# brownvc/matryodshka

Measured on AMD Instinct MI355X. Metric: novel-view frames/sec, 640x320 ODS->32-sphere MSI infer+render, higher is better.
Workload: dtype f32

## Files before the change

include/msi_hip.h:

```cpp
#ifndef MSI_HIP_H
#define MSI_HIP_H

#include <stddef.h>
#include <stdint.h>

#ifdef __cplusplus
extern "C" {
#endif

#define MSI_OK 0
#define MSI_E_BADARG (-1)
#define MSI_E_LAUNCH (-2)
#define MSI_E_UNSUPPORTED (-3)
#define MSI_E_WORKSPACE (-4)
#define MSI_E_RANGE (-5)

typedef void *msi_stream_t;

const char *msi_version(void);
#define MSI_ABI_VERSION 9
int32_t msi_abi_version(void);
const char *msi_last_error_string(void);
uint32_t msi_crc32c_host(const void *data_host, size_t n, uint32_t crc);

// ... 136 lines not shown
#define MSI_NET_OPT_HEAD_FUSE_LN 3
#define MSI_NET_OPT_NUM_CUS 4
#define MSI_NET_OPT_F32_TILE 5
#define MSI_NET_OPT_F32_TILE_MASK 6
#define MSI_NET_OPT_APPLY_AHEAD 7
#define MSI_NET_OPT_HALO 8
#define MSI_NET_OPT_HALO_SKIP 9
#define MSI_NET_OPT_UNIFORM_SPLIT 10
#define MSI_NET_OPT_BF16_STAGE_RAW 11
#define MSI_NET_OPT_SPLIT_OVERHEAD 12
#define MSI_NET_OPT_BF16_WAVES 13
#define MSI_NET_OPT_F32_SPLIT3 14
#define MSI_NET_OPT_F32_SPLIT_F16 15
#define MSI_NET_OPT_X3_TILE8 16
#define MSI_NET_OPT_X3_ROWPAR 17
#define MSI_NET_OPT_COUNT 18
int msi_net_plan_create(const msi_net_desc *desc, msi_net_plan **out_plan);
void msi_net_plan_destroy(msi_net_plan *plan);
int msi_net_plan_set_option(msi_net_plan *plan, int32_t option, int32_t value);
size_t msi_net_plan_workspace_bytes(const msi_net_plan *plan);
int32_t msi_net_plan_layer_is_normalized(const msi_net_plan *plan, int32_t layer);
int32_t msi_net_plan_layer_kernel(const msi_net_plan *plan, int32_t layer, char *name, size_t name_bytes, int32_t *nblocks,
                                  int32_t *nsplit_tiles);
#define MSI_NET_STATUS_APPLY_AHEAD_TIMEOUT 1
#define MSI_NET_STATUS_LN_OVERFLOW 2
#define MSI_NET_STATUS_LN_UNDERFLOW 4
#define MSI_NET_STATUS_F16_SPLIT_RANGE 8
int32_t msi_net_plan_status(const msi_net_plan *plan, const void *workspace, msi_stream_t stream, int32_t *status_bits);
int32_t msi_net_plan_calibrate(const msi_net_plan *plan, float *packed, const void *net_input, void *workspace, size_t workspace_bytes,
                               msi_stream_t stream, int32_t *layers_changed);
int msi_net_plan_forward(const msi_net_plan *plan, const float *packed, const void *net_input, float *pred,
// ... 18 lines not shown
```

matryodshka_amd/_native.py:

```python
import ctypes
import os
from ctypes import POINTER, Structure, c_char, c_char_p, c_float, c_int32, c_size_t, c_uint64, c_void_p

_HERE = os.path.dirname(os.path.abspath(__file__))
LIB_PATH = os.path.join(_HERE, "libmsi_hip.so")

MSI_OK = 0
MSI_NET_NUM_LAYERS = 18
RENDER_STATUS_ORIGIN_OUTSIDE = 1
MSI_CAMERA_EQUIRECT, MSI_CAMERA_PINHOLE = 0, 1
MSI_ABI_VERSION = 9


class MsiError(RuntimeError):
    pass


class NetDesc(Structure):
    _fields_ = [("batch", c_int32), ("height", c_int32), ("width", c_int32),
                ("in_channels", c_int32), ("num_outputs", c_int32), ("ngf", c_int32),
                ("coord_net", c_int32), ("dtype", c_int32)]


MSI_DTYPE_F32, MSI_DTYPE_BF16 = 0, 1
NET_OPT_FIXUP_KERNEL, NET_OPT_TAILSPLIT, NET_OPT_BIGTILE, NET_OPT_HEAD_FUSE_LN, NET_OPT_NUM_CUS = 0, 1, 2, 3, 4
NET_OPT_F32_TILE, NET_OPT_F32_TILE_MASK, NET_OPT_APPLY_AHEAD, NET_OPT_HALO, NET_OPT_HALO_SKIP = 5, 6, 7, 8, 9
NET_OPT_UNIFORM_SPLIT, NET_OPT_BF16_STAGE_RAW, NET_OPT_SPLIT_OVERHEAD, NET_OPT_BF16_WAVES, NET_OPT_F32_SPLIT3 = 10, 11, 12, 13, 14
NET_OPT_F32_SPLIT_F16 = 15
NET_OPT_X3_TILE8 = 16
NET_OPT_X3_ROWPAR = 17
NET_STATUS_F16_SPLIT_RANGE = 8


class LayerInfo(Structure):
    _fields_ = [("name", c_char * 16), ("kind", c_int32), ("cin", c_int32), ("cout", c_int32),
                ("has_coord", c_int32), ("stride", c_int32), ("rate", c_int32),
                ("in_h", c_int32), ("in_w", c_int32), ("out_h", c_int32), ("out_w", c_int32),
                ("param_offset", c_uint64), ("param_floats", c_uint64),
                ("raw_offset", c_uint64), ("affine_offset", c_uint64), ("ln_scale_offset", c_uint64)]


_P = c_void_p
_I = c_int32

SIGNATURES = {
# ... 113 lines not shown
```

matryodshka_amd/csrc/cnn.hip:

```cpp
#include "cnn_device.h"

namespace {

struct Layer {
  char name[16];
  int kind;
  int cin, cout, has_coord, stride, rate;
  int in_h, in_w, out_h, out_w;
  int src0, src1;
  int c0, c1;
  int ntaps, cpt0, cpt1, ksteps, nclass, npad;
  int wrapt;
  int mh, mw;
  double ln_count;
  size_t param_off, param_floats;
  size_t packed_off;
  size_t packed_w_floats;
  size_t gamma_off, beta_off, coord_off;
  size_t lnscl_off;
  size_t x3_off;
  size_t x2_off;
  size_t raw_off, aff_off;
  size_t act_off;
  size_t sums_off;
// ... 298 lines not shown
             (L.rate == 1 || L.rate == 2);
    Q.halo_s2 = halo_ok && (pl->opt[MSI_NET_OPT_HALO] & 4) && !bf16 && !pl->opt[MSI_NET_OPT_APPLY_AHEAD] && Q.tile == TILE_64x64 &&
                L.kind == MODE_CONV && L.stride == 2 && L.rate == 1 && L.src1 < 0 && L.in_h % 2 == 0 && L.in_w % 2 == 0 &&
                L.out_h % 4 == 0 && L.out_w % 16 == 0 && L.c0 % 32 == 0 && p.pad_t == p.pad_l && (p.pad_t == 0 || p.pad_t == 1) &&
                ((long)(L.out_h / 4) * (L.out_w / 16) * (L.cout / 64) * desc->batch >= 3L * pl->num_cus ||
                 (L.x3_off != 0 && ((pl->opt[MSI_NET_OPT_F32_SPLIT3] >> li) & 1) && !(pl->opt[MSI_NET_OPT_HALO_SKIP] >> 20 & 1)));
    if (Q.halo_s2) Q.halo = 1;
    Q.halo_x3 = Q.halo && !bf16 && L.x3_off != 0 && ((pl->opt[MSI_NET_OPT_F32_SPLIT3] >> li) & 1);
    Q.halo_x2 = Q.halo_x3 && ((pl->opt[MSI_NET_OPT_F32_SPLIT_F16] >> li) & 1);
    Q.x3_th8 = Q.halo_x3 && !Q.halo_x2 && !Q.halo_s2 && L.rate == 1 && L.in_h % 8 == 0 && ((pl->opt[MSI_NET_OPT_X3_TILE8] >> li) & 1) &&
               ((long)(L.in_h / 8) * (L.in_w / 16) * ((L.cout + 63) / 64) * desc->batch >= 3L * pl->num_cus || ((pl->opt[MSI_NET_OPT_X3_TILE8] >> 30) & 1));
    if (Q.halo_x3 && !Q.halo_x2 && Q.halo_s2 && L.out_h % 8 == 0 && ((pl->opt[MSI_NET_OPT_X3_TILE8] >> li) & 1) &&
        ((long)(L.out_h / 8) * (L.out_w / 16) * ((L.cout + 63) / 64) * desc->batch >= 3L * pl->num_cus || ((pl->opt[MSI_NET_OPT_X3_TILE8] >> 30) & 1)))
      Q.x3_th8 = 1;
    if (Q.x3_th8) BM = 128;
    p.row_par = (Q.halo_x3 && !Q.halo_s2 && L.kind == MODE_CONV && L.rate == 2 && L.in_h % 8 == 0 && ((pl->opt[MSI_NET_OPT_X3_ROWPAR] >> li) & 1)) ? 1 : 0;
    int max_split = MAX_SPLIT;
    if (halo_ok && (pl->opt[MSI_NET_OPT_HALO] & 1) && bf16 && !pl->opt[MSI_NET_OPT_APPLY_AHEAD] && L.kind == MODE_CONV && L.stride == 1 && L.src1 < 0 && L.in_w % 16 == 0 &&
        L.c0 % 64 == 0 && bigmode != 0) {
      if (L.cout % 128 == 0 && L.in_h % 8 == 0 && (L.rate == 1 || L.rate == 2)) { Q.halo = 1; Q.hbm = 128; Q.hbn = 128; }
      else if (L.cout == 64 && L.in_h % 16 == 0 && L.rate == 1) { Q.halo = 1; Q.hbm = 256; Q.hbn = 64; }
      if (Q.halo) { BM = Q.hbm; BN = Q.hbn; max_split = 1; }
    }
    if (halo_ok && (pl->opt[MSI_NET_OPT_HALO] & 4) && bf16 && !pl->opt[MSI_NET_OPT_APPLY_AHEAD] && L.kind == MODE_CONV && L.stride == 2 && L.rate == 1 &&
        L.src1 < 0 && L.in_h % 2 == 0 && L.in_w % 2 == 0 && L.out_h % 8 == 0 && L.out_w % 16 == 0 && L.c0 % 64 == 0 && L.cout % 128 == 0 &&
        p.pad_t == p.pad_l && (p.pad_t == 0 || p.pad_t == 1) && bigmode != 0) {
      Q.halo = 1; Q.halo_s2 = 1; Q.hbm = 128; Q.hbn = 128; BM = 128; BN = 128; max_split = 1;
    }
    const bool x3_on = !bf16 && L.x3_off != 0 && ((pl->opt[MSI_NET_OPT_F32_SPLIT3] >> li) & 1);
    Q.halo_t = halo_ok && ((pl->opt[MSI_NET_OPT_HALO] & 2) || (x3_on && pl->opt[MSI_NET_OPT_HALO] != 0)) && !bf16
// ... 339 lines not shown
  pl->opt[MSI_NET_OPT_FIXUP_KERNEL] = 0;
  pl->opt[MSI_NET_OPT_TAILSPLIT] = 1;
  pl->opt[MSI_NET_OPT_BIGTILE] = 1;
  pl->opt[MSI_NET_OPT_HEAD_FUSE_LN] = 1;
  pl->opt[MSI_NET_OPT_NUM_CUS] = pl->num_cus;
  pl->opt[MSI_NET_OPT_APPLY_AHEAD] = 0;
  pl->opt[MSI_NET_OPT_HALO] = 5;
  pl->opt[MSI_NET_OPT_F32_TILE] = 0;
  pl->opt[MSI_NET_OPT_F32_TILE_MASK] = 0;
  pl->opt[MSI_NET_OPT_UNIFORM_SPLIT] = 0;
  pl->opt[MSI_NET_OPT_SPLIT_OVERHEAD] = 0;
  pl->opt[MSI_NET_OPT_BF16_WAVES] = 8;
  pl->opt[MSI_NET_OPT_F32_SPLIT_F16] = 0;
  pl->opt[MSI_NET_OPT_X3_TILE8] = 0x3ffff;
  pl->opt[MSI_NET_OPT_X3_ROWPAR] = 0x3ffff;
  pl->opt[MSI_NET_OPT_F32_SPLIT3] = 0x3ffff;
  pl->opt[MSI_NET_OPT_BF16_STAGE_RAW] = 1;
  int rc = plan_layers(pl);
  if (rc) { delete pl; return rc; }
  *out = pl;
  return MSI_OK;
}

void msi_net_plan_destroy(msi_net_plan *plan) { delete plan; }

int msi_net_plan_set_option(msi_net_plan *plan, int32_t option, int32_t value) {
  MSI_REQUIRE(plan, "net_plan_set_option: null plan");
  MSI_REQUIRE(option >= 0 && option < MSI_NET_OPT_COUNT, "net_plan_set_option: unknown option %d", option);
  if (option == MSI_NET_OPT_NUM_CUS) {
    MSI_REQUIRE(value >= 8 && value <= 4096, "net_plan_set_option: num_cus %d out of range", value);
    plan->num_cus = value;
  }
  if (option == MSI_NET_OPT_BIGTILE) MSI_REQUIRE(value >= 0 && value <= 2, "net_plan_set_option: bigtile %d", value);
  if (option == MSI_NET_OPT_HALO) MSI_REQUIRE(value >= 0 && value <= 7, "net_plan_set_option: halo %d (bit 0 conv, bit 1 conv-transpose, bit 2 stride-2 conv)", value);
  if (option == MSI_NET_OPT_TAILSPLIT) MSI_REQUIRE(value >= 0 && value <= 2, "net_plan_set_option: tailsplit %d", value);
  if (option == MSI_NET_OPT_F32_TILE) MSI_REQUIRE(value >= 0 && value <= 2, "net_plan_set_option: f32 tile %d", value);
  if (option == MSI_NET_OPT_BF16_WAVES) MSI_REQUIRE(value == 4 || value == 8, "net_plan_set_option: bf16 waves %d (4 or 8)", value);
#ifndef MSI_EXPERIMENTS
  if ((option == MSI_NET_OPT_F32_TILE || option == MSI_NET_OPT_F32_TILE_MASK || option == MSI_NET_OPT_APPLY_AHEAD) && value != 0)
    return msi::fail(MSI_E_UNSUPPORTED, "net_plan_set_option: option %d is an experiment this library was not built with "
                     "(MSI_CNN_DEFINES=-DMSI_EXPERIMENTS python -m matryodshka_amd.build --force)", option);
#endif
  const int old = plan->opt[option];
  plan->opt[option] = value;
  int rc = plan_layers(plan);
  if (rc) {
    plan->opt[option] = old;
    if (option == MSI_NET_OPT_NUM_CUS) plan->num_cus = old;
    plan_layers(plan);
  }
  return rc;
}
// ... 17 lines not shown
  const int bf16 = plan->desc.dtype == MSI_DTYPE_BF16;
  const char *mode = L.kind == MODE_CONV ? "0" : (L.kind == MODE_CONVT ? "1" : "2");
  if (Q.halo_tb) {
    snprintf(name, name_bytes, "convt_halo_bf16_kernel<128, %d, %d>", Q.hbn, Q.p.halo_apply ? 1 : 0);
  } else if (Q.halo && bf16) {
    if (Q.halo_s2) snprintf(name, name_bytes, "conv_halo_bf16_s2_kernel<%d, 4>", Q.halo_apply ? 1 : 0);
    else if (Q.hbm == 128) snprintf(name, name_bytes, "conv_halo_bf16_kernel<128, 128, %d, %d, %d>", L.rate, Q.halo_apply ? 1 : 0,
                                    plan->opt[MSI_NET_OPT_BF16_WAVES] == 8 ? 8 : 4);
    else snprintf(name, name_bytes, "conv_halo_bf16_kernel<256, 64, 1, %d, 4>", Q.halo_apply ? 1 : 0);
  } else if (Q.halo_t) {
    if (Q.halo_x3 && Q.x3_th8) snprintf(name, name_bytes, "convt_halo8_x3_kernel");
    else if (Q.halo_x3) snprintf(name, name_bytes, "convt_halo_x3_kernel<%d>", Q.halo_x2 ? 2 : 3);
    else snprintf(name, name_bytes, "convt_halo_kernel");
  } else if (Q.halo) {
    if (Q.halo_s2 && Q.halo_x3 && Q.x3_th8) snprintf(name, name_bytes, "conv_halo8_s2_x3_kernel<%d>", Q.halo_apply ? 1 : 0);
    else if (Q.halo_s2 && Q.halo_x3) snprintf(name, name_bytes, "conv_halo_s2_x3_kernel<%d, %d>", Q.halo_apply ? 1 : 0, Q.halo_x2 ? 2 : 3);
    else if (Q.halo_s2) snprintf(name, name_bytes, "conv_halo_s2_kernel<%d>", Q.halo_apply ? 1 : 0);
    else if (Q.x3_th8) snprintf(name, name_bytes, "conv_halo8_x3_kernel<%d, 3>", Q.halo_apply ? 1 : 0);
    else if (Q.halo_x3) snprintf(name, name_bytes, "conv_halo_x3_kernel<%d, %d, %d>", Q.p.row_par ? 3 : L.rate, Q.halo_apply ? 1 : 0, Q.halo_x2 ? 2 : 3);
    else snprintf(name, name_bytes, "conv_halo_kernel<%d, %d>", L.rate, Q.halo_apply ? 1 : 0);
  } else {
    const int bm = Q.tile == TILE_128x128 || Q.tile == TILE_128x64 ? 128 : 64;
    const int bn = Q.tile == TILE_128x128 || Q.tile == TILE_64x128 ? 128 : 64;
    snprintf(name, name_bytes, "conv_igemm_kernel<%d, %d, %s, %d>", bm, bn, mode, bf16);
  }
  if (nblocks) *nblocks = Q.nblocks + Q.p.n_apply;
  if (nsplit_tiles) *nsplit_tiles = Q.nfix;
  return MSI_OK;
}

#ifdef MSI_DEBUG_SUMS
// ... 316 lines not shown
```

matryodshka_amd/csrc/cnn_device.h:

```cpp
#pragma once
#include <cmath>
#include <cstdint>
#include <cstdio>
#include <cstdlib>
#include <cstring>
#include <new>
#include <type_traits>
#include <vector>

#include "msi_common.h"

namespace msi_cnn {


typedef float f32x16 __attribute__((ext_vector_type(16)));
typedef float v4f __attribute__((ext_vector_type(4)));
typedef __attribute__((address_space(3))) void lds_void;

constexpr int BK = 32;
constexpr int ROW_BYTES = BK * 4;
#ifndef MSI_NSTAGE
#define MSI_NSTAGE 2
#endif
constexpr int NSTAGE = MSI_NSTAGE;
constexpr int NPAD_ALIGN = 128;
constexpr int COORD_CLASSES = 5;
[[maybe_unused]] constexpr unsigned OOB = 0x80000000u;
constexpr int DEFAULT_CUS = 256;
constexpr int MAX_SPLIT = 8;
constexpr int CONV_SLOTS_PER_CU = 5;
constexpr double LN_EPS = 1e-12;
constexpr int LN_SHARDS = 64, LN_WORDS = 2;
constexpr int LN_S1_BITS = 24, LN_S2_BITS = 16;
constexpr int LN_SCL_DOUBLES = 4;
constexpr double LN_UNDERFLOW_UNITS_SQ = 1e12;
enum { STATUS_APPLY_AHEAD_TIMEOUT = 1, STATUS_LN_OVERFLOW = 2, STATUS_LN_UNDERFLOW = 4, STATUS_F16_SPLIT_RANGE = 8 };
constexpr int AP_FLAG_STRIDE = 16;
constexpr int HEAD_MAX_C = 256;

enum { MODE_CONV = 0, MODE_CONVT = 1, MODE_HEAD = 2 };

struct ConvParams {
  const char *x0, *x1;
  const char *wpk;
// ... 45 lines not shown

enum { TILE_64x64 = 0, TILE_128x128 = 1, TILE_128x64 = 2, TILE_64x128 = 3 };

struct LayerLaunch {
  ConvParams p;
  int tile;
  int nblocks, nfix;
  int inlaunch;
  int fuse_ln;
  int skip_apply;
  int halo;
  int halo_s2;
  int halo_x3;
  int halo_x2;
  int x3_th8;
  int hbm, hbn;
  int halo_t;
  int halo_tb;
  int halo_apply;
  unsigned ln_blocks;
};


constexpr int HA_TP = 32;
#ifndef MSI_HA_LG
#define MSI_HA_LG 32
#endif
constexpr int HA_LG = MSI_HA_LG;

struct HeadAsmParams {
// ... 681 lines not shown
```

matryodshka_amd/csrc/cnn_x3.hip:

```cpp
#include "cnn_device.h"

namespace {

#ifndef MSI_X3_EARLY_DMA
#define MSI_X3_EARLY_DMA 0
#endif
#ifndef MSI_X3_NSTG
#define MSI_X3_NSTG 0
#endif
#ifndef MSI_X3_ABLATE
#define MSI_X3_ABLATE 0
#endif
#ifndef MSI_X2_NSTG
#define MSI_X2_NSTG 3
#endif
constexpr int x3_rate_y(int RATE) { return RATE == 3 ? 1 : RATE; }
constexpr int x3_rate_x(int RATE) { return RATE == 3 ? 2 : RATE; }
constexpr int x3_nstg(int RATE, int NPL) { return NPL == 2 ? MSI_X2_NSTG : (MSI_X3_NSTG ? MSI_X3_NSTG : (RATE == 2 ? 3 : 2)); }
template <int RATE, int NS = x3_nstg(RATE, 3), int NPL = 3, int TH = 4>
struct HaloGeomX3 {
  static constexpr int PW = 16 + 2 * x3_rate_x(RATE), PH = TH + 2 * x3_rate_y(RATE), NPX = PW * PH;
  static constexpr int PIX_BYTES = NPL * 64 + 16;
  static constexpr int ROW_PITCH = ((PW * PIX_BYTES + 127) / 256) * 256 + 128;
  static constexpr int A_BYTES = PH * ROW_PITCH;
// ... 408 lines not shown
    v4f r = y - v4f{__builtin_bit_cast(float, h0 << 16), __builtin_bit_cast(float, h0 & 0xffff0000u),
                    __builtin_bit_cast(float, h1 << 16), __builtin_bit_cast(float, h1 & 0xffff0000u)};
    asm("v_cvt_pk_bf16_f32 %0, %1, %2" : "=v"(m0) : "v"(r.x), "v"(r.y));
    asm("v_cvt_pk_bf16_f32 %0, %1, %2" : "=v"(m1) : "v"(r.z), "v"(r.w));
    r = r - v4f{__builtin_bit_cast(float, m0 << 16), __builtin_bit_cast(float, m0 & 0xffff0000u),
                __builtin_bit_cast(float, m1 << 16), __builtin_bit_cast(float, m1 & 0xffff0000u)};
    asm("v_cvt_pk_bf16_f32 %0, %1, %2" : "=v"(l0) : "v"(r.x), "v"(r.y));
    asm("v_cvt_pk_bf16_f32 %0, %1, %2" : "=v"(l1) : "v"(r.z), "v"(r.w));
    if (off != 0xffffffffu) {
      *reinterpret_cast<u2x_t *>(smem + off) = u2x_t{h0, h1};
      *reinterpret_cast<u2x_t *>(smem + off + 64) = u2x_t{m0, m1};
      *reinterpret_cast<u2x_t *>(smem + off + 128) = u2x_t{l0, l1};
    }
  }
}
template <int NP>
__device__ __forceinline__ void split_mfma(f32x16 &acc, f32x16 &lo, const v4f &ah, const v4f &am, const v4f &al, const v4f &bh, const v4f &bm, const v4f &bl) {
  typedef __bf16 bf16x8 __attribute__((ext_vector_type(8)));
  typedef _Float16 f16x8 __attribute__((ext_vector_type(8)));
  if (NP == 2) {
    lo = __builtin_amdgcn_mfma_f32_32x32x16_f16(__builtin_bit_cast(f16x8, bm), __builtin_bit_cast(f16x8, ah), lo, 0, 0, 0);
    acc = __builtin_amdgcn_mfma_f32_32x32x16_f16(__builtin_bit_cast(f16x8, bh), __builtin_bit_cast(f16x8, ah), acc, 0, 0, 0);
    lo = __builtin_amdgcn_mfma_f32_32x32x16_f16(__builtin_bit_cast(f16x8, bh), __builtin_bit_cast(f16x8, am), lo, 0, 0, 0);
  } else {
    acc = __builtin_amdgcn_mfma_f32_32x32x16_bf16(__builtin_bit_cast(bf16x8, bm), __builtin_bit_cast(bf16x8, am), acc, 0, 0, 0);
    acc = __builtin_amdgcn_mfma_f32_32x32x16_bf16(__builtin_bit_cast(bf16x8, bh), __builtin_bit_cast(bf16x8, al), acc, 0, 0, 0);
    acc = __builtin_amdgcn_mfma_f32_32x32x16_bf16(__builtin_bit_cast(bf16x8, bl), __builtin_bit_cast(bf16x8, ah), acc, 0, 0, 0);
    acc = __builtin_amdgcn_mfma_f32_32x32x16_bf16(__builtin_bit_cast(bf16x8, bh), __builtin_bit_cast(bf16x8, am), acc, 0, 0, 0);
    acc = __builtin_amdgcn_mfma_f32_32x32x16_bf16(__builtin_bit_cast(bf16x8, bm), __builtin_bit_cast(bf16x8, ah), acc, 0, 0, 0);
    acc = __builtin_amdgcn_mfma_f32_32x32x16_bf16(__builtin_bit_cast(bf16x8, bh), __builtin_bit_cast(bf16x8, ah), acc, 0, 0, 0);
  }
}
template <int NP>
__device__ __forceinline__ void split_finish(f32x16 &acc, const f32x16 &lo, unsigned amax, int lane, int *status) {
  if (NP == 2) {
#pragma unroll
    for (int r = 0; r < 16; ++r) acc[r] = __builtin_fmaf(lo[r], 1.f / 2048.f, acc[r]);
    if (__builtin_amdgcn_ballot_w64(amax > F16_MAX_BITS) != 0 && lane == 0) atomicOr(status, STATUS_F16_SPLIT_RANGE);
  }
}

#ifndef MSI_S2X3_NSTG
#define MSI_S2X3_NSTG 2
#endif
template <int NP, int TH = 4>
struct HaloGeomS2X3 {
  static constexpr int PW = 17, PH = TH + 1, NPX = PW * PH;
  static constexpr int PIX_BYTES = NP * 64 + 16;
  static constexpr int ROW_PITCH = ((PW * PIX_BYTES + 127) / 256) * 256 + 128;
  static constexpr int A_BYTES = PH * ROW_PITCH;
  static constexpr int B_ROW = 64, B_PLANE = 64 * B_ROW, B_STAGE = NP * B_PLANE;
  static constexpr int NSTG = NP == 3 ? MSI_S2X3_NSTG : 3;
  static constexpr int LDS_BYTES = A_BYTES + NSTG * B_STAGE;
  static constexpr int NLOAD = (NPX * 8 + 255) / 256;
};

#ifndef MSI_S2X_WAVES
#define MSI_S2X_WAVES 3
#ifndef MSI_S2X3_ABLATE
#define MSI_S2X3_ABLATE 0
#endif
#endif
template <int APPLY, int NP, int TH>
__device__ __forceinline__ void conv_halo_s2_x3_body(const ConvParams &p, char *smem) {
  typedef HaloGeomS2X3<NP, TH> G;
  constexpr int PW = G::PW, NPX = G::NPX, NLOAD = G::NLOAD;
  constexpr int MT = TH / 4, NT = 1, BM = 16 * TH;
  static_assert(TH == 4 || (TH == 8 && NP == 3 && G::NSTG == 2), "the 8-row tile: six-product form, two-stage ring");
  const int tid = threadIdx.x, lane = tid & 63;
  const int wave = __builtin_amdgcn_readfirstlane(tid >> 6);
  const int wm = wave >> 1, wn = wave & 1;
  const int CH = p.cpt0;
  int t, c0 = 0, c1 = CH, ks = 0, slot = 0;
  {
    const int bid = blockIdx.x;
    if (bid < p.nb_main && p.split0 == 1) {
      const int q = p.n_main >> 3, r = p.n_main & 7, xcd = bid & 7, local = bid >> 3;
      t = (xcd < r ? xcd * (q + 1) : r * (q + 1) + (xcd - r) * q) + local;
    } else {
      int sp, r, tbase;
      unsigned mg;
      if (bid < p.nb_main) { sp = p.split0; mg = p.mg_sp0; r = bid; tbase = 0; }
      else { sp = p.split; mg = p.mg_sp; r = bid - p.nb_main; tbase = p.n_main; }
// ... 63 lines not shown
      }
      __builtin_amdgcn_sched_barrier(0);
    }
  }

  float inv_f = 1.f, mu_hi = 0.f, mu_lo = 0.f;
  bool has_pad = false;
  if (APPLY) {
    bool bad = false;
#pragma unroll
    for (int k = 0; k < NLOAD; ++k)
#pragma unroll
      for (int u = 0; u < 4; ++u) bad |= (lds_a[k] != 0xffffffffu) && !pok[u][k];
    has_pad = __builtin_amdgcn_ballot_w64(bad) != 0;
  }
  v4f s4 = {1.f, 1.f, 1.f, 1.f}, t4 = {0.f, 0.f, 0.f, 0.f};
  auto patch_load = [&](const int c, auto U_c) __attribute__((always_inline)) {
    constexpr int U = decltype(U_c)::value;
    if (MSI_S2X3_ABLATE & 64) return;
#pragma unroll
    for (int k_ = 0; k_ < NLOAD; ++k_)
      araw[k_] = __builtin_bit_cast(v4f, (u32x4_t)__builtin_amdgcn_raw_buffer_load_b128(rsrc_a, voff[U][k_], c * ROW_BYTES, 0));
    if (APPLY && U == 0) {
      g4 = *reinterpret_cast<const v4f *>(p.ln_gamma + c * 32 + cslot * 4);
      be4 = *reinterpret_cast<const v4f *>(p.ln_beta + c * 32 + cslot * 4);
    }
  };
  auto patch_store = [&](auto U_c) __attribute__((always_inline)) {
    constexpr int U = decltype(U_c)::value;
    if (APPLY && U == 0) {
      s4 = inv_f * g4;
      const v4f nh = {-mu_hi, -mu_hi, -mu_hi, -mu_hi}, nl = {-mu_lo, -mu_lo, -mu_lo, -mu_lo};
      t4 = __builtin_elementwise_fma(nl, s4, __builtin_elementwise_fma(nh, s4, be4));
    }
#pragma unroll
    for (int k_ = 0; k_ < NLOAD; ++k_) {
      v4f y = araw[k_];
      if (APPLY) {
        y = __builtin_elementwise_max(__builtin_elementwise_fma(y, s4, t4), v4f{0.f, 0.f, 0.f, 0.f});
        if (has_pad && !pok[U][k_]) y = v4f{0.f, 0.f, 0.f, 0.f};
      }
// ... 12 lines not shown
  typedef __bf16 bf16x8 __attribute__((ext_vector_type(8), unused));
  f32x16 acc[MT][1], acc_lo;
#pragma unroll
  for (int r = 0; r < 16; ++r) {
    acc_lo[r] = 0.f;
#pragma unroll
    for (int i = 0; i < MT; ++i) acc[i][0][r] = 0.f;
  }

  int c = c0, cpar = 0;
  auto s2step = [&](auto J_c) __attribute__((always_inline)) {
    constexpr int J = decltype(J_c)::value;
    constexpr int TAP_ = s2_tap(J), U_ = s2_unit(J);
    constexpr int DY_ = (TAP_ / 3) >> 1, DX_ = (TAP_ % 3) >> 1;
    constexpr bool FIRST_ = J == 0 || J == 4 || J == 6 || J == 8, LAST_ = J == 3 || J == 5 || J == 7 || J == 8;
    constexpr int AOFF_ = DY_ * G::ROW_PITCH + DX_ * G::PIX_BYTES;
    const bool more_ = U_ < 3 || c + 1 < c1;
    const unsigned bst_ = (unsigned)(G::NSTG == 3 ? J % 3 : ((J ^ cpar) & 1)) * G::B_STAGE;
    if (G::NSTG == 2) {
      const int stn_ = ((J ^ cpar) & 1) ^ 1;
      if (J + 1 < 9) b_issue(c, s2_tap((J + 1) % 9), stn_);
      else if (c + 1 < c1) b_issue(c + 1, s2_tap(0), stn_);
    }
    v4f ah_[2], am_[2], al_[2], bh_[2], bm_[2], bl_[2];
    if constexpr (MT == 2) {
      constexpr int A1_ = AOFF_ + 2 * G::ROW_PITCH;
      v4f xh_[2][2], xm_[2][2], xl_[2][2];
      bh_[0] = lds_read128<0>(b_s[0] + bst_); bm_[0] = lds_read128<G::B_PLANE>(b_s[0] + bst_); bl_[0] = lds_read128<2 * G::B_PLANE>(b_s[0] + bst_);
      xh_[0][0] = lds_read128<AOFF_>(a_base); xm_[0][0] = lds_read128<AOFF_ + 64>(a_base); xl_[0][0] = lds_read128<AOFF_ + 128>(a_base);
      xh_[0][1] = lds_read128<A1_>(a_base); xm_[0][1] = lds_read128<A1_ + 64>(a_base); xl_[0][1] = lds_read128<A1_ + 128>(a_base);
      bh_[1] = lds_read128<0>(b_s[1] + bst_); bm_[1] = lds_read128<G::B_PLANE>(b_s[1] + bst_); bl_[1] = lds_read128<2 * G::B_PLANE>(b_s[1] + bst_);
      wait_lgkm6<6>(bh_[0], bm_[0], bl_[0], xh_[0][0], xm_[0][0], xl_[0][0]);
// ... 15 lines not shown
      split_mfma<3>(acc[1][0], acc_lo, xh_[1][1], xm_[1][1], xl_[1][1], bh_[1], bm_[1], bl_[1]);
      __builtin_amdgcn_sched_barrier(0);
    } else {
    if (!(MSI_S2X3_ABLATE & 8))
#pragma unroll
    for (int s_ = 0; s_ < 2; ++s_) {
      ah_[s_] = s_ == 0 ? lds_read128<AOFF_>(a_base) : lds_read128<AOFF_ + 32>(a_base);
      bh_[s_] = lds_read128<0>(b_s[s_] + bst_);
      am_[s_] = s_ == 0 ? lds_read128<AOFF_ + 64>(a_base) : lds_read128<AOFF_ + 96>(a_base);
      bm_[s_] = lds_read128<G::B_PLANE>(b_s[s_] + bst_);
      if (NP == 3) {
        al_[s_] = s_ == 0 ? lds_read128<AOFF_ + 128>(a_base) : lds_read128<AOFF_ + 160>(a_base);
        bl_[s_] = lds_read128<2 * G::B_PLANE>(b_s[s_] + bst_);
      } else { al_[s_] = ah_[s_]; bl_[s_] = bh_[s_]; }
    }
#pragma unroll
    for (int s_ = 0; s_ < 2; ++s_) {
      if (NP == 3) {
        if (s_ == 0) wait_lgkm6<6>(ah_[0], bh_[0], am_[0], bm_[0], al_[0], bl_[0]);
        else wait_lgkm6<0>(ah_[1], bh_[1], am_[1], bm_[1], al_[1], bl_[1]);
      } else {
        if (s_ == 0) wait_lgkm4<4>(ah_[0], bh_[0], am_[0], bm_[0]);
        else wait_lgkm4<0>(ah_[1], bh_[1], am_[1], bm_[1]);
      }
      if (!(MSI_S2X3_ABLATE & 16)) split_mfma<NP>(acc[0][0], acc_lo, ah_[s_], am_[s_], al_[s_], bh_[s_], bm_[s_], bl_[s_]);
      __builtin_amdgcn_sched_barrier(0);
      if (s_ == 0) {
        if (FIRST_ && more_) {
          if (U_ < 3) patch_load(c, IC<(U_ + 1) & 3>{});
          else patch_load(c + 1, IC<0>{});
        }
        if (G::NSTG == 3) {
        if (J + 2 < 9) b_issue(c, s2_tap((J + 2) % 9), (J + 2) % 3);
        else if (c + 1 < c1) b_issue(c + 1, s2_tap((J + 2) % 9), (J + 2) % 3);
        }
      }
    }
    }
    {
      const bool issued_ = (J + 2 < 9) || (c + 1 < c1);
      if (G::NSTG == 2) {
        if (FIRST_ && !LAST_ && more_) wait_vmcnt<NLOAD>();
        else wait_vmcnt<0>();
      } else if (FIRST_ && !LAST_ && more_) wait_vmcnt<NP + NLOAD>();
      else if (issued_) wait_vmcnt<NP>();
      else wait_vmcnt<0>();
    }
    if (!(MSI_S2X3_ABLATE & 4)) __builtin_amdgcn_s_barrier();
    if (LAST_ && more_ && !(MSI_S2X3_ABLATE & 32)) {
      patch_store(IC<(U_ + 1) & 3>{});
      asm volatile("s_waitcnt lgkmcnt(0)" ::: "memory");
      __builtin_amdgcn_s_barrier();
    }
  };

  if (APPLY) {
    double *s_stat = reinterpret_cast<double *>(smem);
    ln_mean_inv(p.ln_sums + (size_t)b * LN_SHARDS * LN_WORDS, p.ln_inv_n, p.ln_scl_src, p.status, s_stat, tid);
    const double mu = s_stat[0];
    inv_f = (float)s_stat[1];
    mu_hi = (float)mu;
    mu_lo = (float)(mu - (double)mu_hi);
    __syncthreads();
  }
  wait_vmcnt<0>();
  patch_store(IC<0>{});
  asm volatile("s_waitcnt lgkmcnt(0)" ::: "memory");
  __builtin_amdgcn_s_barrier();
  for (; c < c1; ++c) {
    cpar = (c - c0) & 1;
    s2step(IC<0>{}); s2step(IC<1>{}); s2step(IC<2>{}); s2step(IC<3>{}); s2step(IC<4>{});
    s2step(IC<5>{}); s2step(IC<6>{}); s2step(IC<7>{}); s2step(IC<8>{});
  }
  split_finish<NP>(acc[0][0], acc_lo, amax_, lane, p.status);

  if (!full) {
    constexpr int SLAB = BM * 64 * 4;
    const __amdgpu_buffer_rsrc_t rsrc_p = __builtin_amdgcn_make_buffer_rsrc((void *)(p.partial + (size_t)slot * (BM * 64)), 0, SLAB, 0x00020000);
    if (p.tile_cnt == nullptr) {
      dump_acc<MT, NT, 0>(acc, rsrc_p, tid);
      return;
// ... 9 lines not shown
    __syncthreads();
    if (*s_old != nsp - 1) return;
    handoff_acquire();
    const __amdgpu_buffer_rsrc_t rsrc_t = __builtin_amdgcn_make_buffer_rsrc((void *)(p.partial + (size_t)(slot - ks) * (BM * 64)), 0, nsp * SLAB, 0x00020000);
    sum_slabs<MT, NT, MSI_HANDOFF_AUX>(acc, rsrc_t, nsp, SLAB, tid);
    __syncthreads();
  }
  emit_tile<BM, 64, MODE_CONV>(p, acc, tile_m, tile_n, 0, b, tid, smem);
}

template <int APPLY, int NP>
__global__ void __launch_bounds__(256) __attribute__((amdgpu_waves_per_eu(NP == 2 ? MSI_S2X_WAVES : (MSI_S2X3_NSTG == 2 ? 3 : 2))))
conv_halo_s2_x3_kernel(const ConvParams p) {
#if defined(__HIP_DEVICE_COMPILE__)
  extern __shared__ __attribute__((aligned(16))) char smem[];
  conv_halo_s2_x3_body<APPLY, NP, 4>(p, smem);
#endif
}

template <int APPLY>
__global__ void __launch_bounds__(256) __attribute__((amdgpu_waves_per_eu(2)))
conv_halo8_s2_x3_kernel(const ConvParams p) {
#if defined(__HIP_DEVICE_COMPILE__)
  extern __shared__ __attribute__((aligned(16))) char smem[];
  conv_halo_s2_x3_body<APPLY, 3, 8>(p, smem);
#endif
}

template <int NS, int NPL, int TH = 4>
struct HaloGeomCT3 : HaloGeomX3<1, NS, NPL, TH> {
  typedef HaloGeomX3<1, NS, NPL, TH> B_;
// ... 336 lines not shown
  convt_halo_x3_body<3, 8>(p, smem);
#endif
}

}

namespace msi_cnn {
int launch_x3(const LayerLaunch &Q, const ConvParams &p, int rate, hipStream_t stream) {
  const dim3 grid(Q.nblocks), block(256);
  if (Q.halo_t) {
    constexpr int lds_ct3 = HaloGeomCT3<MSI_CT3_NSTG, 3>::LDS_BYTES, lds_ct2 = HaloGeomCT3<3, 2>::LDS_BYTES;
    constexpr int lds_ct8 = HaloGeomCT3<MSI_CT3_NSTG, 3, 8>::LDS_BYTES;
    static_assert(lds_ct8 <= 65536, "convt_halo8_x3_kernel: LDS without the launch attribute");
    if (Q.x3_th8) hipLaunchKernelGGL(convt_halo8_x3_kernel, grid, block, lds_ct8, stream, p);
    else if (Q.halo_x2) hipLaunchKernelGGL(convt_halo_x3_kernel<2>, grid, block, lds_ct2, stream, p);
    else hipLaunchKernelGGL(convt_halo_x3_kernel<3>, grid, block, lds_ct3, stream, p);
    int rc = msi::check_launch("convt_halo_x3");
    if (!rc && Q.nfix > 0 && p.tile_cnt == nullptr) rc = launch_fixup(Q.x3_th8 ? 128 : 64, 64, MODE_CONVT, Q.nfix, 2, p, stream);
    return rc;
  }
  if (Q.halo_s2 && Q.x3_th8) {
    typedef HaloGeomS2X3<3, 8> G8s_;
    static_assert(G8s_::LDS_BYTES <= 65536, "conv_halo8_s2_x3_kernel: LDS without the launch attribute");
    if (Q.halo_apply) hipLaunchKernelGGL((conv_halo8_s2_x3_kernel<1>), grid, block, G8s_::LDS_BYTES, stream, p);
    else hipLaunchKernelGGL((conv_halo8_s2_x3_kernel<0>), grid, block, G8s_::LDS_BYTES, stream, p);
  } else if (Q.halo_s2) {
    if (Q.halo_x2) {
      if (Q.halo_apply) hipLaunchKernelGGL((conv_halo_s2_x3_kernel<1, 2>), grid, block, HaloGeomS2X3<2>::LDS_BYTES, stream, p);
      else hipLaunchKernelGGL((conv_halo_s2_x3_kernel<0, 2>), grid, block, HaloGeomS2X3<2>::LDS_BYTES, stream, p);
    } else {
      if (Q.halo_apply) hipLaunchKernelGGL((conv_halo_s2_x3_kernel<1, 3>), grid, block, HaloGeomS2X3<3>::LDS_BYTES, stream, p);
      else hipLaunchKernelGGL((conv_halo_s2_x3_kernel<0, 3>), grid, block, HaloGeomS2X3<3>::LDS_BYTES, stream, p);
    }
  } else if (Q.x3_th8) {
    typedef HaloGeomX3<1, (MSI_X3_NSTG ? MSI_X3_NSTG : 2), 3, 8> G8_;
    static_assert(G8_::LDS_BYTES <= 65536, "conv_halo8_x3_kernel: LDS without the launch attribute");
    if (Q.halo_apply) hipLaunchKernelGGL((conv_halo8_x3_kernel<1, 3>), grid, block, G8_::LDS_BYTES, stream, p);
    else hipLaunchKernelGGL((conv_halo8_x3_kernel<0, 3>), grid, block, G8_::LDS_BYTES, stream, p);
  } else {
    static thread_local unsigned long long done2[12] = {0};
#define MSI_X3_LAUNCH(R, A, N)                                                                                         \
  {                                                                                                                    \
    typedef HaloGeomX3<R, x3_nstg(R, N), N> G_;                                                                        \
    if (G_::LDS_BYTES > 65536) {                                                                                       \
      int rc0 = set_max_lds(reinterpret_cast<const void *>(conv_halo_x3_kernel<R, A, N>), G_::LDS_BYTES, done2[(R - 1) * 4 + A * 2 + (N - 2)], "conv_halo_x3"); \
      if (rc0) return rc0;                                                                                             \
    }                                                                                                                  \
    hipLaunchKernelGGL((conv_halo_x3_kernel<R, A, N>), grid, block, G_::LDS_BYTES, stream, p);                          \
  }
    const int sel = (rate == 1 ? 0 : (p.row_par ? 8 : 4)) + (Q.halo_apply ? 2 : 0) + (Q.halo_x2 ? 0 : 1);
    switch (sel) {
      case 0: MSI_X3_LAUNCH(1, 0, 2) break;
      case 1: MSI_X3_LAUNCH(1, 0, 3) break;
      case 2: MSI_X3_LAUNCH(1, 1, 2) break;
      case 3: MSI_X3_LAUNCH(1, 1, 3) break;
      case 4: MSI_X3_LAUNCH(2, 0, 2) break;
      case 5: MSI_X3_LAUNCH(2, 0, 3) break;
      case 6: MSI_X3_LAUNCH(2, 1, 2) break;
      case 7: MSI_X3_LAUNCH(2, 1, 3) break;
      case 8: MSI_X3_LAUNCH(3, 0, 2) break;
      case 9: MSI_X3_LAUNCH(3, 0, 3) break;
      case 10: MSI_X3_LAUNCH(3, 1, 2) break;
      default: MSI_X3_LAUNCH(3, 1, 3) break;
// ... 9 lines not shown
```

Measured before the change: 544.6.

## Pre-split the next patch during MFMAs in the stride-2 x3 halo kernel

```diff
diff --git a/include/msi_hip.h b/include/msi_hip.h
--- a/include/msi_hip.h
+++ b/include/msi_hip.h
@@ -174,7 +174,8 @@
 #define MSI_NET_OPT_F32_SPLIT_F16 15
 #define MSI_NET_OPT_X3_TILE8 16
 #define MSI_NET_OPT_X3_ROWPAR 17
-#define MSI_NET_OPT_COUNT 18
+#define MSI_NET_OPT_X3_DBUF 18
+#define MSI_NET_OPT_COUNT 19
 int msi_net_plan_create(const msi_net_desc *desc, msi_net_plan **out_plan);
 void msi_net_plan_destroy(msi_net_plan *plan);
 int msi_net_plan_set_option(msi_net_plan *plan, int32_t option, int32_t value);
diff --git a/matryodshka_amd/_native.py b/matryodshka_amd/_native.py
--- a/matryodshka_amd/_native.py
+++ b/matryodshka_amd/_native.py
@@ -29,6 +29,7 @@
 NET_OPT_F32_SPLIT_F16 = 15
 NET_OPT_X3_TILE8 = 16
 NET_OPT_X3_ROWPAR = 17
+NET_OPT_X3_DBUF = 18
 NET_STATUS_F16_SPLIT_RANGE = 8
 
 
diff --git a/matryodshka_amd/csrc/cnn.hip b/matryodshka_amd/csrc/cnn.hip
--- a/matryodshka_amd/csrc/cnn.hip
+++ b/matryodshka_amd/csrc/cnn.hip
@@ -336,6 +336,7 @@
         ((long)(L.out_h / 8) * (L.out_w / 16) * ((L.cout + 63) / 64) * desc->batch >= 3L * pl->num_cus || ((pl->opt[MSI_NET_OPT_X3_TILE8] >> 30) & 1)))
       Q.x3_th8 = 1;
     if (Q.x3_th8) BM = 128;
+    Q.x3_dbuf = (Q.halo_s2 && Q.halo_x3 && !Q.halo_x2 && !Q.x3_th8 && ((pl->opt[MSI_NET_OPT_X3_DBUF] >> li) & 1)) ? 1 : 0;
     p.row_par = (Q.halo_x3 && !Q.halo_s2 && L.kind == MODE_CONV && L.rate == 2 && L.in_h % 8 == 0 && ((pl->opt[MSI_NET_OPT_X3_ROWPAR] >> li) & 1)) ? 1 : 0;
     int max_split = MAX_SPLIT;
     if (halo_ok && (pl->opt[MSI_NET_OPT_HALO] & 1) && bf16 && !pl->opt[MSI_NET_OPT_APPLY_AHEAD] && L.kind == MODE_CONV && L.stride == 1 && L.src1 < 0 && L.in_w % 16 == 0 &&
@@ -705,6 +706,7 @@
   pl->opt[MSI_NET_OPT_F32_SPLIT_F16] = 0;
   pl->opt[MSI_NET_OPT_X3_TILE8] = 0x3ffff;
   pl->opt[MSI_NET_OPT_X3_ROWPAR] = 0x3ffff;
+  pl->opt[MSI_NET_OPT_X3_DBUF] = X3_DBUF_S2_DEFAULT ? 0x3ffff : 0;
   pl->opt[MSI_NET_OPT_F32_SPLIT3] = 0x3ffff;
   pl->opt[MSI_NET_OPT_BF16_STAGE_RAW] = 1;
   int rc = plan_layers(pl);
@@ -727,6 +729,7 @@
   if (option == MSI_NET_OPT_TAILSPLIT) MSI_REQUIRE(value >= 0 && value <= 2, "net_plan_set_option: tailsplit %d", value);
   if (option == MSI_NET_OPT_F32_TILE) MSI_REQUIRE(value >= 0 && value <= 2, "net_plan_set_option: f32 tile %d", value);
   if (option == MSI_NET_OPT_BF16_WAVES) MSI_REQUIRE(value == 4 || value == 8, "net_plan_set_option: bf16 waves %d (4 or 8)", value);
+  if (option == MSI_NET_OPT_X3_DBUF) MSI_REQUIRE((value & ~0x3ffff) == 0, "net_plan_set_option: x3 dbuf 0x%x (one bit per layer, 18 layers)", value);
 #ifndef MSI_EXPERIMENTS
   if ((option == MSI_NET_OPT_F32_TILE || option == MSI_NET_OPT_F32_TILE_MASK || option == MSI_NET_OPT_APPLY_AHEAD) && value != 0)
     return msi::fail(MSI_E_UNSUPPORTED, "net_plan_set_option: option %d is an experiment this library was not built with "
@@ -774,7 +777,8 @@
     else snprintf(name, name_bytes, "convt_halo_kernel");
   } else if (Q.halo) {
     if (Q.halo_s2 && Q.halo_x3 && Q.x3_th8) snprintf(name, name_bytes, "conv_halo8_s2_x3_kernel<%d>", Q.halo_apply ? 1 : 0);
-    else if (Q.halo_s2 && Q.halo_x3) snprintf(name, name_bytes, "conv_halo_s2_x3_kernel<%d, %d>", Q.halo_apply ? 1 : 0, Q.halo_x2 ? 2 : 3);
+    else if (Q.halo_s2 && Q.halo_x3) snprintf(name, name_bytes, "conv_halo_s2_x3_kernel<%d, %d>%s", Q.halo_apply ? 1 : 0, Q.halo_x2 ? 2 : 3,
+                                              Q.halo_x2 || (Q.x3_dbuf != 0) == X3_DBUF_S2_DEFAULT ? "" : (Q.x3_dbuf ? " [dbuf]" : " [1buf]"));
     else if (Q.halo_s2) snprintf(name, name_bytes, "conv_halo_s2_kernel<%d>", Q.halo_apply ? 1 : 0);
     else if (Q.x3_th8) snprintf(name, name_bytes, "conv_halo8_x3_kernel<%d, 3>", Q.halo_apply ? 1 : 0);
     else if (Q.halo_x3) snprintf(name, name_bytes, "conv_halo_x3_kernel<%d, %d, %d>", Q.p.row_par ? 3 : L.rate, Q.halo_apply ? 1 : 0, Q.halo_x2 ? 2 : 3);
diff --git a/matryodshka_amd/csrc/cnn_device.h b/matryodshka_amd/csrc/cnn_device.h
--- a/matryodshka_amd/csrc/cnn_device.h
+++ b/matryodshka_amd/csrc/cnn_device.h
@@ -28,6 +28,10 @@
 [[maybe_unused]] constexpr unsigned OOB = 0x80000000u;
 constexpr int DEFAULT_CUS = 256;
 constexpr int MAX_SPLIT = 8;
+#ifndef MSI_X3_DBUF_S2
+#define MSI_X3_DBUF_S2 0
+#endif
+constexpr bool X3_DBUF_S2_DEFAULT = MSI_X3_DBUF_S2 != 0;
 constexpr int CONV_SLOTS_PER_CU = 5;
 constexpr double LN_EPS = 1e-12;
 constexpr int LN_SHARDS = 64, LN_WORDS = 2;
@@ -103,6 +107,7 @@
   int halo_x3;
   int halo_x2;
   int x3_th8;
+  int x3_dbuf;
   int hbm, hbn;
   int halo_t;
   int halo_tb;
diff --git a/matryodshka_amd/csrc/cnn_x3.hip b/matryodshka_amd/csrc/cnn_x3.hip
--- a/matryodshka_amd/csrc/cnn_x3.hip
+++ b/matryodshka_amd/csrc/cnn_x3.hip
@@ -8,6 +8,10 @@
 #ifndef MSI_X3_NSTG
 #define MSI_X3_NSTG 0
 #endif
+#ifndef MSI_X3_LDS_FLOOR
+#define MSI_X3_LDS_FLOOR 0
+#endif
+constexpr int x3_lds(int bytes) { return bytes < MSI_X3_LDS_FLOOR ? MSI_X3_LDS_FLOOR : bytes; }
 #ifndef MSI_X3_ABLATE
 #define MSI_X3_ABLATE 0
 #endif
@@ -446,6 +450,24 @@
     }
   }
 }
+__device__ __forceinline__ void split3_parts(v4f y, unsigned &h0, unsigned &h1, unsigned &m0, unsigned &m1, unsigned &l0, unsigned &l1) {
+  asm("v_cvt_pk_bf16_f32 %0, %1, %2" : "=v"(h0) : "v"(y.x), "v"(y.y));
+  asm("v_cvt_pk_bf16_f32 %0, %1, %2" : "=v"(h1) : "v"(y.z), "v"(y.w));
+  v4f r = y - v4f{__builtin_bit_cast(float, h0 << 16), __builtin_bit_cast(float, h0 & 0xffff0000u),
+                  __builtin_bit_cast(float, h1 << 16), __builtin_bit_cast(float, h1 & 0xffff0000u)};
+  asm("v_cvt_pk_bf16_f32 %0, %1, %2" : "=v"(m0) : "v"(r.x), "v"(r.y));
+  asm("v_cvt_pk_bf16_f32 %0, %1, %2" : "=v"(m1) : "v"(r.z), "v"(r.w));
+  r = r - v4f{__builtin_bit_cast(float, m0 << 16), __builtin_bit_cast(float, m0 & 0xffff0000u),
+              __builtin_bit_cast(float, m1 << 16), __builtin_bit_cast(float, m1 & 0xffff0000u)};
+  asm("v_cvt_pk_bf16_f32 %0, %1, %2" : "=v"(l0) : "v"(r.x), "v"(r.y));
+  asm("v_cvt_pk_bf16_f32 %0, %1, %2" : "=v"(l1) : "v"(r.z), "v"(r.w));
+}
+__device__ __forceinline__ void store3_parts(char *smem, unsigned off, unsigned h0, unsigned h1, unsigned m0, unsigned m1, unsigned l0, unsigned l1) {
+  typedef unsigned u2x_t __attribute__((ext_vector_type(2)));
+  *reinterpret_cast<u2x_t *>(smem + off) = u2x_t{h0, h1};
+  *reinterpret_cast<u2x_t *>(smem + off + 64) = u2x_t{m0, m1};
+  *reinterpret_cast<u2x_t *>(smem + off + 128) = u2x_t{l0, l1};
+}
 template <int NP>
 __device__ __forceinline__ void split_mfma(f32x16 &acc, f32x16 &lo, const v4f &ah, const v4f &am, const v4f &al, const v4f &bh, const v4f &bm, const v4f &bl) {
   typedef __bf16 bf16x8 __attribute__((ext_vector_type(8)));
@@ -475,30 +497,38 @@
 #ifndef MSI_S2X3_NSTG
 #define MSI_S2X3_NSTG 2
 #endif
-template <int NP, int TH = 4>
+template <int NP, int TH = 4, int NBUF = 1>
 struct HaloGeomS2X3 {
   static constexpr int PW = 17, PH = TH + 1, NPX = PW * PH;
   static constexpr int PIX_BYTES = NP * 64 + 16;
   static constexpr int ROW_PITCH = ((PW * PIX_BYTES + 127) / 256) * 256 + 128;
-  static constexpr int A_BYTES = PH * ROW_PITCH;
+  static constexpr int A_BUF = PH * ROW_PITCH, A_BYTES = NBUF * A_BUF;
+  static constexpr int A_DUMP = PW * PIX_BYTES - 16;
+  static_assert(A_DUMP >= (PW - 1) * PIX_BYTES + NP * 64 && A_DUMP + NP * 64 <= ROW_PITCH, "the dump slot lies in bytes of row 0 that nobody reads");
   static constexpr int B_ROW = 64, B_PLANE = 64 * B_ROW, B_STAGE = NP * B_PLANE;
   static constexpr int NSTG = NP == 3 ? MSI_S2X3_NSTG : 3;
   static constexpr int LDS_BYTES = A_BYTES + NSTG * B_STAGE;
   static constexpr int NLOAD = (NPX * 8 + 255) / 256;
 };
 
+#ifndef MSI_S2X3_PRESPLIT
+#define MSI_S2X3_PRESPLIT 1
+#endif
 #ifndef MSI_S2X_WAVES
 #define MSI_S2X_WAVES 3
 #ifndef MSI_S2X3_ABLATE
 #define MSI_S2X3_ABLATE 0
 #endif
 #endif
-template <int APPLY, int NP, int TH>
+template <int APPLY, int NP, int TH, int NBUF = 1, bool PRE = false>
 __device__ __forceinline__ void conv_halo_s2_x3_body(const ConvParams &p, char *smem) {
-  typedef HaloGeomS2X3<NP, TH> G;
+  typedef HaloGeomS2X3<NP, TH, NBUF> G;
   constexpr int PW = G::PW, NPX = G::NPX, NLOAD = G::NLOAD;
   constexpr int MT = TH / 4, NT = 1, BM = 16 * TH;
+  constexpr bool DB = NBUF == 2 || PRE;
+  static_assert(!PRE || (NBUF == 1 && NP == 3 && TH == 4 && G::NSTG == 2), "split ahead of the swap: the 4-row six-product form on the two-stage ring");
   static_assert(TH == 4 || (TH == 8 && NP == 3 && G::NSTG == 2), "the 8-row tile: six-product form, two-stage ring");
+  static_assert(NBUF == 1 || (NBUF == 2 && NP == 3 && TH == 4 && G::NSTG == 2), "two patch buffers: the 4-row six-product form on the two-stage ring");
   const int tid = threadIdx.x, lane = tid & 63;
   const int wave = __builtin_amdgcn_readfirstlane(tid >> 6);
   const int wm = wave >> 1, wn = wave & 1;
@@ -592,6 +622,11 @@
       for (int u = 0; u < 4; ++u) bad |= (lds_a[k] != 0xffffffffu) && !pok[u][k];
     has_pad = __builtin_amdgcn_ballot_w64(bad) != 0;
   }
+  if (DB) {
+#pragma unroll
+    for (int k = 0; k < NLOAD; ++k)
+      if (lds_a[k] == 0xffffffffu) lds_a[k] = (unsigned)(G::A_DUMP + cslot * 8);
+  }
   v4f s4 = {1.f, 1.f, 1.f, 1.f}, t4 = {0.f, 0.f, 0.f, 0.f};
   auto patch_load = [&](const int c, auto U_c) __attribute__((always_inline)) {
     constexpr int U = decltype(U_c)::value;
@@ -599,10 +634,39 @@
 #pragma unroll
     for (int k_ = 0; k_ < NLOAD; ++k_)
       araw[k_] = __builtin_bit_cast(v4f, (u32x4_t)__builtin_amdgcn_raw_buffer_load_b128(rsrc_a, voff[U][k_], c * ROW_BYTES, 0));
-    if (APPLY && U == 0) {
+    if (APPLY && U == 0 && !DB) {
       g4 = *reinterpret_cast<const v4f *>(p.ln_gamma + c * 32 + cslot * 4);
       be4 = *reinterpret_cast<const v4f *>(p.ln_beta + c * 32 + cslot * 4);
     }
+  };
+  unsigned parts[NLOAD][6];
+  auto affine_load = [&](const int c) __attribute__((always_inline)) {
+    if (!APPLY || (MSI_S2X3_ABLATE & 64)) return;
+    g4 = *reinterpret_cast<const v4f *>(p.ln_gamma + c * 32 + cslot * 4);
+    be4 = *reinterpret_cast<const v4f *>(p.ln_beta + c * 32 + cslot * 4);
+  };
+  auto patch_pieces = [&](auto U_c, auto K0_c, auto K1_c) __attribute__((always_inline)) {
+    constexpr int U = decltype(U_c)::value, K0 = decltype(K0_c)::value, K1 = decltype(K1_c)::value;
+    if (APPLY && U == 0 && K0 == 0) {
+      s4 = inv_f * g4;
+      const v4f nh = {-mu_hi, -mu_hi, -mu_hi, -mu_hi}, nl = {-mu_lo, -mu_lo, -mu_lo, -mu_lo};
+      t4 = __builtin_elementwise_fma(nl, s4, __builtin_elementwise_fma(nh, s4, be4));
+    }
+#pragma unroll
+    for (int k_ = K0; k_ < K1; ++k_) {
+      v4f y = araw[k_];
+      if (APPLY) {
+        y = __builtin_elementwise_max(__builtin_elementwise_fma(y, s4, t4), v4f{0.f, 0.f, 0.f, 0.f});
+        if (has_pad && !pok[U][k_]) y = v4f{0.f, 0.f, 0.f, 0.f};
+      }
+      split3_parts(y, parts[k_][0], parts[k_][1], parts[k_][2], parts[k_][3], parts[k_][4], parts[k_][5]);
+      if (!PRE) store3_parts(smem + (U & 1) * G::A_BUF, lds_a[k_], parts[k_][0], parts[k_][1], parts[k_][2], parts[k_][3], parts[k_][4], parts[k_][5]);
+    }
+  };
+  auto parts_to_lds = [&]() __attribute__((always_inline)) {
+#pragma unroll
+    for (int k_ = 0; k_ < NLOAD; ++k_)
+      store3_parts(smem, lds_a[k_], parts[k_][0], parts[k_][1], parts[k_][2], parts[k_][3], parts[k_][4], parts[k_][5]);
   };
   auto patch_store = [&](auto U_c) __attribute__((always_inline)) {
     constexpr int U = decltype(U_c)::value;
@@ -645,8 +709,10 @@
     constexpr int TAP_ = s2_tap(J), U_ = s2_unit(J);
     constexpr int DY_ = (TAP_ / 3) >> 1, DX_ = (TAP_ % 3) >> 1;
     constexpr bool FIRST_ = J == 0 || J == 4 || J == 6 || J == 8, LAST_ = J == 3 || J == 5 || J == 7 || J == 8;
-    constexpr int AOFF_ = DY_ * G::ROW_PITCH + DX_ * G::PIX_BYTES;
+    constexpr int AOFF_ = DY_ * G::ROW_PITCH + DX_ * G::PIX_BYTES + (NBUF == 2 ? (U_ & 1) * G::A_BUF : 0);
+    constexpr int NH_ = (NLOAD + 1) / 2;
     const bool more_ = U_ < 3 || c + 1 < c1;
+    if (DB && J == 6 && c + 1 < c1) affine_load(c + 1);
     const unsigned bst_ = (unsigned)(G::NSTG == 3 ? J % 3 : ((J ^ cpar) & 1)) * G::B_STAGE;
     if (G::NSTG == 2) {
       const int stn_ = ((J ^ cpar) & 1) ^ 1;
@@ -692,6 +758,7 @@
         bl_[s_] = lds_read128<2 * G::B_PLANE>(b_s[s_] + bst_);
       } else { al_[s_] = ah_[s_]; bl_[s_] = bh_[s_]; }
     }
+    if (DB && LAST_) __builtin_amdgcn_sched_barrier(0);
 #pragma unroll
     for (int s_ = 0; s_ < 2; ++s_) {
       if (NP == 3) {
@@ -702,9 +769,16 @@
         else wait_lgkm4<0>(ah_[1], bh_[1], am_[1], bm_[1]);
       }
       if (!(MSI_S2X3_ABLATE & 16)) split_mfma<NP>(acc[0][0], acc_lo, ah_[s_], am_[s_], al_[s_], bh_[s_], bm_[s_], bl_[s_]);
-      __builtin_amdgcn_sched_barrier(0);
+      if constexpr (DB) {
+        if (LAST_ && !(MSI_S2X3_ABLATE & 32)) {
+          if (s_ == 0) patch_pieces(IC<(U_ + 1) & 3>{}, IC<0>{}, IC<NH_>{});
+          else patch_pieces(IC<(U_ + 1) & 3>{}, IC<NH_>{}, IC<NLOAD>{});
+        }
+      }
+      __builtin_amdgcn_sched_barrier(0);
+      if (DB && J == 7 && s_ == 1 && c + 1 < c1) patch_load(c + 1, IC<0>{});
       if (s_ == 0) {
-        if (FIRST_ && more_) {
+        if (FIRST_ && more_ && !(DB && LAST_)) {
           if (U_ < 3) patch_load(c, IC<(U_ + 1) & 3>{});
           else patch_load(c + 1, IC<0>{});
         }
@@ -717,7 +791,11 @@
     }
     {
       const bool issued_ = (J + 2 < 9) || (c + 1 < c1);
-      if (G::NSTG == 2) {
+      if (DB) {
+        if ((FIRST_ && !LAST_) || (J == 7 && c + 1 < c1)) wait_vmcnt<NLOAD>();
+        else wait_vmcnt<0>();
+        if (LAST_ && !PRE) asm volatile("s_waitcnt lgkmcnt(0)" ::: "memory");
+      } else if (G::NSTG == 2) {
         if (FIRST_ && !LAST_ && more_) wait_vmcnt<NLOAD>();
         else wait_vmcnt<0>();
       } else if (FIRST_ && !LAST_ && more_) wait_vmcnt<NP + NLOAD>();
@@ -725,7 +803,12 @@
       else wait_vmcnt<0>();
     }
     if (!(MSI_S2X3_ABLATE & 4)) __builtin_amdgcn_s_barrier();
-    if (LAST_ && more_ && !(MSI_S2X3_ABLATE & 32)) {
+    if (PRE && LAST_ && more_ && !(MSI_S2X3_ABLATE & 32)) {
+      parts_to_lds();
+      asm volatile("s_waitcnt lgkmcnt(0)" ::: "memory");
+      __builtin_amdgcn_s_barrier();
+    }
+    if (!DB && LAST_ && more_ && !(MSI_S2X3_ABLATE & 32)) {
       patch_store(IC<(U_ + 1) & 3>{});
       asm volatile("s_waitcnt lgkmcnt(0)" ::: "memory");
       __builtin_amdgcn_s_barrier();
@@ -742,7 +825,8 @@
     __syncthreads();
   }
   wait_vmcnt<0>();
-  patch_store(IC<0>{});
+  if constexpr (DB) { patch_pieces(IC<0>{}, IC<0>{}, IC<NLOAD>{}); if (PRE) parts_to_lds(); }
+  else patch_store(IC<0>{});
   asm volatile("s_waitcnt lgkmcnt(0)" ::: "memory");
   __builtin_amdgcn_s_barrier();
   for (; c < c1; ++c) {
@@ -782,7 +866,16 @@
 conv_halo_s2_x3_kernel(const ConvParams p) {
 #if defined(__HIP_DEVICE_COMPILE__)
   extern __shared__ __attribute__((aligned(16))) char smem[];
-  conv_halo_s2_x3_body<APPLY, NP, 4>(p, smem);
+  conv_halo_s2_x3_body<APPLY, NP, 4, 1, (NP == 3 && MSI_S2X3_PRESPLIT != 0 && MSI_S2X3_NSTG == 2)>(p, smem);
+#endif
+}
+
+template <int APPLY>
+__global__ void __launch_bounds__(256) __attribute__((amdgpu_waves_per_eu(2)))
+conv_halo_s2_x3_db_kernel(const ConvParams p) {
+#if defined(__HIP_DEVICE_COMPILE__)
+  extern __shared__ __attribute__((aligned(16))) char smem[];
+  conv_halo_s2_x3_body<APPLY, 3, 4, 2>(p, smem);
 #endif
 }
 
@@ -1149,7 +1242,7 @@
     static_assert(lds_ct8 <= 65536, "convt_halo8_x3_kernel: LDS without the launch attribute");
     if (Q.x3_th8) hipLaunchKernelGGL(convt_halo8_x3_kernel, grid, block, lds_ct8, stream, p);
     else if (Q.halo_x2) hipLaunchKernelGGL(convt_halo_x3_kernel<2>, grid, block, lds_ct2, stream, p);
-    else hipLaunchKernelGGL(convt_halo_x3_kernel<3>, grid, block, lds_ct3, stream, p);
+    else hipLaunchKernelGGL(convt_halo_x3_kernel<3>, grid, block, x3_lds(lds_ct3), stream, p);
     int rc = msi::check_launch("convt_halo_x3");
     if (!rc && Q.nfix > 0 && p.tile_cnt == nullptr) rc = launch_fixup(Q.x3_th8 ? 128 : 64, 64, MODE_CONVT, Q.nfix, 2, p, stream);
     return rc;
@@ -1163,9 +1256,14 @@
     if (Q.halo_x2) {
       if (Q.halo_apply) hipLaunchKernelGGL((conv_halo_s2_x3_kernel<1, 2>), grid, block, HaloGeomS2X3<2>::LDS_BYTES, stream, p);
       else hipLaunchKernelGGL((conv_halo_s2_x3_kernel<0, 2>), grid, block, HaloGeomS2X3<2>::LDS_BYTES, stream, p);
+    } else if (Q.x3_dbuf) {
+      typedef HaloGeomS2X3<3, 4, 2> Gd_;
+      static_assert(Gd_::LDS_BYTES <= 65536, "conv_halo_s2_x3_db_kernel: LDS without the launch attribute");
+      if (Q.halo_apply) hipLaunchKernelGGL((conv_halo_s2_x3_db_kernel<1>), grid, block, Gd_::LDS_BYTES, stream, p);
+      else hipLaunchKernelGGL((conv_halo_s2_x3_db_kernel<0>), grid, block, Gd_::LDS_BYTES, stream, p);
     } else {
-      if (Q.halo_apply) hipLaunchKernelGGL((conv_halo_s2_x3_kernel<1, 3>), grid, block, HaloGeomS2X3<3>::LDS_BYTES, stream, p);
-      else hipLaunchKernelGGL((conv_halo_s2_x3_kernel<0, 3>), grid, block, HaloGeomS2X3<3>::LDS_BYTES, stream, p);
+      if (Q.halo_apply) hipLaunchKernelGGL((conv_halo_s2_x3_kernel<1, 3>), grid, block, x3_lds(HaloGeomS2X3<3>::LDS_BYTES), stream, p);
+      else hipLaunchKernelGGL((conv_halo_s2_x3_kernel<0, 3>), grid, block, x3_lds(HaloGeomS2X3<3>::LDS_BYTES), stream, p);
     }
   } else if (Q.x3_th8) {
     typedef HaloGeomX3<1, (MSI_X3_NSTG ? MSI_X3_NSTG : 2), 3, 8> G8_;
@@ -1181,7 +1279,7 @@
       int rc0 = set_max_lds(reinterpret_cast<const void *>(conv_halo_x3_kernel<R, A, N>), G_::LDS_BYTES, done2[(R - 1) * 4 + A * 2 + (N - 2)], "conv_halo_x3"); \
       if (rc0) return rc0;                                                                                             \
     }                                                                                                                  \
-    hipLaunchKernelGGL((conv_halo_x3_kernel<R, A, N>), grid, block, G_::LDS_BYTES, stream, p);                          \
+    hipLaunchKernelGGL((conv_halo_x3_kernel<R, A, N>), grid, block, N == 3 ? x3_lds(G_::LDS_BYTES) : G_::LDS_BYTES, stream, p); \
   }
     const int sel = (rate == 1 ? 0 : (p.row_par ? 8 : 4)) + (Q.halo_apply ? 2 : 0) + (Q.halo_x2 ? 0 : 1);
     switch (sel) {
```

New measurement: 543.7, median of 2. No clear change (-0.2%).
